# microsoft/ptgnn

Hardware: AMD Instinct MI355X
Metric: edges/sec per MP layer (higher is better)
Workload: dtype f32; 1 GPU; cfg3: Graph2Class-style batch, 48 graphs N=115772, T0=8->T=17, E=625130 (incl. reverse+self), Typilus GGNN arch: 8 GGNN layers H=128 (+concat residual), max; hidden=128, mode=forward (inference), fp32, plan_build_in_step=True, message_rows=shared per (edge type, source) pair, parallelism=single GPU, minibatches_rotated=4

## Files before the change

include/ptgnn_amd.h:

```cpp
#ifndef PTGNN_AMD_H_
#define PTGNN_AMD_H_

#include <stddef.h>
#include <stdint.h>

#ifdef __cplusplus
extern "C" {
#endif

#pragma GCC visibility push(default)

#define PTGNN_AMD_VERSION 102

enum {
  PTGNN_AMD_OK = 0,
  PTGNN_AMD_EINVAL = -1,
  PTGNN_AMD_EUNSUPPORTED = -2,
  PTGNN_AMD_EHIP = -3,
  PTGNN_AMD_EWORKSPACE = -4,
  PTGNN_AMD_ERANGE = -5
};

enum { PTGNN_AMD_SUM = 0, PTGNN_AMD_MEAN = 1, PTGNN_AMD_MAX = 2, PTGNN_AMD_MIN = 3 };

// ... 103 lines not shown
int64_t ptgnn_amd_hub_ticket_count(int64_t num_edges, int32_t msg_dim);
int ptgnn_amd_gather_reduce_f32(const float *ysrc, int64_t ld_ysrc,
                                const float *ydst , int64_t ld_ydst,
                                const int32_t *rowptr, const int32_t *col,
                                int32_t type_bits, int64_t num_nodes, int32_t msg_dim,
                                int reduce, int epilogue, const float *ln_gamma,
                                const float *ln_beta, float ln_eps, float *out, int64_t ld_out,
                                int32_t *argout , int64_t num_edges,
                                int32_t hub_threshold, const int32_t *hub_entries ,
                                const int32_t *hub_count , void *hub_ws ,
                                size_t hub_ws_bytes, int32_t *hub_tickets ,
                                void *stream);
int ptgnn_amd_gather_reduce_rows_f32(const float *ysrc, int64_t ld_ysrc,
                                     const float *ydst , int64_t ld_ydst,
                                     const int32_t *rowptr, const int32_t *col,
                                     int32_t type_bits, int64_t num_nodes, int32_t msg_dim,
                                     int reduce, int epilogue, const float *ln_gamma,
                                     const float *ln_beta, float ln_eps, float *out, int64_t ld_out,
                                     int32_t *argout , int64_t num_edges,
                                     int32_t hub_threshold, const int32_t *hub_entries ,
                                     const int32_t *hub_count , void *hub_ws ,
                                     size_t hub_ws_bytes, int32_t *hub_tickets ,
                                     int64_t row_begin, int64_t row_end, void *stream);

int ptgnn_amd_gather_update_supported(int32_t msg_dim, int32_t out_dim);
int ptgnn_amd_gather_update_f32(const float *msg, int64_t ld_msg, const int32_t *rowptr, const int32_t *col,
                                int32_t type_bits, int64_t num_nodes, int32_t msg_dim, int reduce, int epilogue,
                                const float *ln_gamma , const float *ln_beta , float ln_eps,
                                const float *w , const float *bias ,
                                int32_t out_dim, int act, float *out, int64_t ld_out, void *stream);

int ptgnn_amd_segment_mul_f32(const float *msg, int64_t ld_msg, const int32_t *rowptr, const int32_t *perm,
                              int64_t num_rows, int64_t num_edges, int32_t dim, float *out, int64_t ld_out,
                              void *stream);

int ptgnn_amd_gather_reduce_masked_f32(const float *grad, int64_t ld_grad, const int32_t *arg,
                                       const int32_t *rowptr, const int32_t *col,
                                       const int32_t *slot_of, int64_t num_rows, int32_t msg_dim,
                                       float *out, int64_t ld_out, int64_t num_edges,
                                       int32_t hub_threshold, const int32_t *hub_entries,
                                       const int32_t *hub_count, void *hub_ws ,
                                       size_t hub_ws_bytes, int32_t *hub_tickets ,
                                       void *stream);

int ptgnn_amd_linear_f32(const float *x, int64_t rows, int32_t k, int64_t ld_x, const float *w,
                         int32_t n_out, const float *bias, int act, float *y, int64_t ld_y,
// ... 250 lines not shown
```

ptgnn_amd/_lib.py:

```python
import ctypes
import os
import threading

import torch

_HERE = os.path.dirname(os.path.abspath(__file__))
LIB_PATH = os.environ.get("PTGNN_AMD_LIB") or os.path.join(_HERE, "csrc", "libptgnn_amd.so")

_c = ctypes
_i64, _i32, _vp, _f32 = _c.c_int64, _c.c_int32, _c.c_void_p, _c.c_float

SIGNATURES = {
    "ptgnn_amd_version": (_c.c_int, []),
    "ptgnn_amd_last_error": (_c.c_char_p, []),
    "ptgnn_amd_set_gemm_mode": (_c.c_int, [_c.c_int]),
    "ptgnn_amd_get_gemm_mode": (_c.c_int, []),
    "ptgnn_amd_launch_count": (_i64, [_c.c_int]),
    "ptgnn_amd_launch_name": (_c.c_char_p, [_c.c_int]),
    "ptgnn_amd_csr_workspace_bytes": (_c.c_size_t, [_i64, _i64]),
    "ptgnn_amd_csr_control_bytes": (_c.c_size_t, []),
    "ptgnn_amd_set_plan_path": (_c.c_int, [_c.c_int]),
    "ptgnn_amd_type_bits": (_c.c_int, [_i32]),
    "ptgnn_amd_csr_build": (_c.c_int, [_vp, _vp, _vp, _i32, _i64, _i64, _c.c_int, _vp, _vp, _vp, _vp,
                                       _i32, _vp, _vp, _vp, _vp, _vp, _c.c_size_t, _vp]),
    "ptgnn_amd_hub_workspace_bytes": (_c.c_size_t, [_i64, _i32, _c.c_int]),
    "ptgnn_amd_hub_ticket_count": (_i64, [_i64, _i32]),
    "ptgnn_amd_hub_list": (_c.c_int, [_vp, _i64, _i32, _vp, _vp, _vp]),
    "ptgnn_amd_validate_indices": (_c.c_int, [_vp, _i64, _i64, _vp, _vp]),
    "ptgnn_amd_shard_index_workspace_bytes": (_c.c_size_t, [_i64]),
    "ptgnn_amd_shard_index": (_c.c_int, [_vp, _vp, _vp, _i32, _i64, _i64, _vp, _i32, _i64, _vp, _vp, _vp, _i64, _vp,
                                         _vp, _vp, _c.c_size_t, _vp]),
    "ptgnn_amd_unique_sources_workspace_bytes": (_c.c_size_t, [_i64, _i32]),
    "ptgnn_amd_edge_table_bytes": (_c.c_size_t, []),
    "ptgnn_amd_unique_sources": (_c.c_int, [_vp, _i64, _i32, _i32, _i64, _vp, _vp, _i64, _vp, _vp, _vp, _c.c_size_t,
                                            _vp]),
    "ptgnn_amd_edge_linear_shared_supported": (_c.c_int, [_i32, _i32, _i32]),
    "ptgnn_amd_edge_linear_shared_f32": (_c.c_int, [_vp, _i64, _i64, _i32, _vp, _vp, _i32, _i32, _c.c_int, _vp, _i64,
                                                    _vp]),
    "ptgnn_amd_gather_reduce_f32": (_c.c_int, [_vp, _i64, _vp, _i64, _vp, _vp, _i32, _i64, _i32, _c.c_int,
                                               _c.c_int, _vp, _vp, _f32, _vp, _i64, _vp, _i64, _i32, _vp,
                                               _vp, _vp, _c.c_size_t, _vp, _vp]),
    "ptgnn_amd_gather_reduce_rows_f32": (_c.c_int, [_vp, _i64, _vp, _i64, _vp, _vp, _i32, _i64, _i32, _c.c_int,
                                                    _c.c_int, _vp, _vp, _f32, _vp, _i64, _vp, _i64, _i32, _vp,
                                                    _vp, _vp, _c.c_size_t, _vp, _i64, _i64, _vp]),
    "ptgnn_amd_gather_update_supported": (_c.c_int, [_i32, _i32]),
    "ptgnn_amd_gather_update_f32": (_c.c_int, [_vp, _i64, _vp, _vp, _i32, _i64, _i32, _c.c_int, _c.c_int, _vp, _vp, _f32,
                                               _vp, _vp, _i32, _c.c_int, _vp, _i64, _vp]),
    "ptgnn_amd_gather_reduce_masked_f32": (_c.c_int, [_vp, _i64, _vp, _vp, _vp, _vp, _i64, _i32, _vp, _i64,
                                                      _i64, _i32, _vp, _vp, _vp, _c.c_size_t, _vp, _vp]),
    "ptgnn_amd_segment_mul_f32": (_c.c_int, [_vp, _i64, _vp, _vp, _i64, _i64, _i32, _vp, _i64, _vp]),
    "ptgnn_amd_linear_f32": (_c.c_int, [_vp, _i64, _i32, _i64, _vp, _i32, _vp, _c.c_int, _vp, _i64,
                                        _vp]),
    "ptgnn_amd_linear_add_f32": (_c.c_int, [_vp, _i64, _i32, _i64, _vp, _i32, _vp, _c.c_int, _vp, _i64, _vp, _i64,
                                            _vp]),
    "ptgnn_amd_batch_offsets_i64": (_c.c_int, [_vp, _i64, _vp, _vp, _i32, _i64, _vp, _vp]),
    "ptgnn_amd_edge_linear_f32": (_c.c_int, [_vp, _i64, _i64, _i32, _vp, _vp, _vp, _vp, _i32, _i32, _c.c_int, _vp,
                                             _i64, _vp]),
    "ptgnn_amd_edge_linear_feat_f32": (_c.c_int, [_vp, _i64, _i64, _i32, _vp, _vp, _vp, _i64, _i32, _vp, _vp, _i32, _i32,
                                                  _c.c_int, _vp, _i64, _vp]),
    "ptgnn_amd_edge_linear_dropout_f32": (_c.c_int, [_vp, _i64, _i64, _i32, _vp, _vp, _vp, _i32, _i32, _vp, _i64,
                                                     _c.c_int, _c.c_float, _c.c_uint64, _vp]),
    "ptgnn_amd_dropout_bitmask_bytes": (_c.c_size_t, [_i64, _i32]),
    "ptgnn_amd_dropout_bitmask": (_c.c_int, [_i64, _i32, _c.c_float, _c.c_uint64, _vp, _vp]),
    "ptgnn_amd_edge_linear_masked_supported": (_c.c_int, [_i32, _i32, _c.c_int]),
    "ptgnn_amd_edge_linear_masked_f32": (_c.c_int, [_vp, _i64, _i64, _i32, _vp, _vp, _vp, _i32, _i32, _vp, _i64,
                                                    _c.c_int, _c.c_float, _vp, _vp]),
    "ptgnn_amd_edge_weight_grad_masked_supported": (_c.c_int, [_i32, _i32]),
# ... 128 lines not shown
```

ptgnn_amd/csrc/gather_reduce.hip:

```cpp
#include "gather_reduce_core.h"

namespace ptgnn_amd {
namespace {
constexpr int kSidePool = 64;
std::mutex g_side_mu;
SideStream g_side[kSidePool];
int g_side_used = 0;

bool side_streams_enabled() {
  static const bool enabled = [] {
    const char *e = getenv("PTGNN_AMD_HUB_STREAM");
    return !(e && e[0] == '0');
  }();
  return enabled;
}
}

SideStream *side_stream(hipStream_t caller, bool may_create) {
  if (!side_streams_enabled()) return nullptr;
  int dev = 0;
  if (hipGetDevice(&dev) != hipSuccess) return nullptr;
  std::lock_guard<std::mutex> lock(g_side_mu);
  for (int i = 0; i < g_side_used; ++i)
    if (g_side[i].dev == dev && g_side[i].owner == caller) return &g_side[i];
// ... 121 lines not shown
                                           int32_t type_bits, int64_t num_nodes, int32_t msg_dim,
                                           int reduce, int epilogue, const float *ln_gamma,
                                           const float *ln_beta, float ln_eps, float *out,
                                           int64_t ld_out, int32_t *argout, int64_t num_edges,
                                           int32_t hub_threshold, const int32_t *hub_entries,
                                           const int32_t *hub_count, void *hub_ws,
                                           size_t hub_ws_bytes, int32_t *hub_tickets, void *stream_) {
  return ptgnn_amd_gather_reduce_rows_f32(ysrc, ld_y, ydst, ld_yd, rowptr, col, type_bits, num_nodes, msg_dim, reduce,
                                          epilogue, ln_gamma, ln_beta, ln_eps, out, ld_out, argout, num_edges,
                                          hub_threshold, hub_entries, hub_count, hub_ws, hub_ws_bytes, hub_tickets, 0,
                                          num_nodes, stream_);
}

extern "C" int ptgnn_amd_gather_reduce_rows_f32(const float *ysrc, int64_t ld_y, const float *ydst,
                                                int64_t ld_yd, const int32_t *rowptr, const int32_t *col,
                                                int32_t type_bits, int64_t num_nodes, int32_t msg_dim,
                                                int reduce, int epilogue, const float *ln_gamma,
                                                const float *ln_beta, float ln_eps, float *out,
                                                int64_t ld_out, int32_t *argout, int64_t num_edges,
                                                int32_t hub_threshold, const int32_t *hub_entries,
                                                const int32_t *hub_count, void *hub_ws,
                                                size_t hub_ws_bytes, int32_t *hub_tickets, int64_t row_begin,
                                                int64_t row_end, void *stream_) {
  hipStream_t stream = (hipStream_t)stream_;
  PTGNN_REQUIRE(num_nodes >= 0 && msg_dim > 0 && num_edges >= 0, PTGNN_AMD_EINVAL, "gather_reduce: bad sizes");
  PTGNN_REQUIRE(row_begin >= 0 && row_begin <= row_end && row_end <= num_nodes, PTGNN_AMD_EINVAL,
                "gather_reduce: row range [%lld, %lld) outside [0, %lld]", (long long)row_begin, (long long)row_end,
                (long long)num_nodes);
  if (row_begin == row_end) return PTGNN_AMD_OK;
  PTGNN_REQUIRE(reduce >= PTGNN_AMD_SUM && reduce <= PTGNN_AMD_MIN, PTGNN_AMD_EINVAL,
                "gather_reduce: unknown reduce %d", reduce);
  PTGNN_REQUIRE(epilogue >= 0 && epilogue <= 3, PTGNN_AMD_EINVAL, "gather_reduce: bad epilogue");
  PTGNN_REQUIRE(type_bits >= 0 && type_bits < 16, PTGNN_AMD_EINVAL, "gather_reduce: bad type_bits");
  if (num_nodes == 0) return PTGNN_AMD_OK;
  PTGNN_REQUIRE(rowptr && out && ld_out >= msg_dim, PTGNN_AMD_EINVAL, "gather_reduce: null/ld");
  PTGNN_REQUIRE(col && (ysrc || num_edges == 0), PTGNN_AMD_EINVAL, "gather_reduce: null ysrc/col");
  PTGNN_REQUIRE(!(epilogue & PTGNN_AMD_EPI_LAYERNORM) || (ln_gamma && ln_beta), PTGNN_AMD_EINVAL,
                "gather_reduce: LayerNorm epilogue needs gamma/beta");
  PTGNN_REQUIRE(argout == nullptr || reduce >= PTGNN_AMD_MAX, PTGNN_AMD_EINVAL,
                "gather_reduce: argout only with max/min");

  Args a{};
  a.ysrc = ysrc; a.ydst = ydst; a.ld_y = ld_y; a.ld_yd = ydst ? ld_yd : ld_y;
  a.rowptr = rowptr; a.col = col; a.type_bits = type_bits; a.num_nodes = row_end; a.row_begin = row_begin; a.msg_dim = msg_dim;
  a.ln_gamma = ln_gamma; a.ln_beta = ln_beta; a.ln_eps = ln_eps; a.out = out; a.ld_out = ld_out;
  a.argout = argout; a.epi = epilogue;
  const int rc = setup_hub(a, num_edges, hub_threshold, hub_entries, hub_count, hub_ws, hub_ws_bytes,
                           hub_tickets, argout != nullptr);
  if (rc != PTGNN_AMD_OK) return rc;
  const bool vec4 = (msg_dim % 4 == 0) && (ld_y % 4 == 0) && (!ydst || ld_yd % 4 == 0) && (ld_out % 4 == 0) &&
                    aligned16(ysrc) && aligned16(out) && (!ydst || aligned16(ydst)) &&
                    (!argout || aligned16(argout));
  const bool row_epi = (epilogue & PTGNN_AMD_EPI_LAYERNORM) != 0;
  const int rc2 = dispatch_geometry(vec4, msg_dim, row_epi, [&](auto V, auto L, auto C, int col_blocks) {
    return launch1<decltype(V)::value, decltype(L)::value, decltype(C)::value>(a, reduce, col_blocks, stream);
  });
  if (rc2 == PTGNN_AMD_OK) count_launch(PTGNN_AMD_KERNEL_GATHER_REDUCE);
  return rc2;
}

extern "C" int ptgnn_amd_gather_update_supported(int32_t msg_dim, int32_t out_dim) {
  return msg_dim == kUpdM && out_dim >= 32 && out_dim <= 128 && out_dim % 32 == 0 ? 1 : 0;
}

extern "C" int ptgnn_amd_gather_update_f32(const float *msg, int64_t ld_msg, const int32_t *rowptr, const int32_t *col,
                                           int32_t type_bits, int64_t num_nodes, int32_t msg_dim, int reduce,
                                           int epilogue, const float *ln_gamma, const float *ln_beta, float ln_eps,
                                           const float *w, const float *bias, int32_t out_dim, int act, float *out,
                                           int64_t ld_out, void *stream_) {
// ... 45 lines not shown
  hipStream_t stream = (hipStream_t)stream_;
  PTGNN_REQUIRE(num_rows >= 0 && msg_dim > 0 && num_edges >= 0, PTGNN_AMD_EINVAL,
                "gather_reduce_masked: bad sizes");
  if (num_rows == 0) return PTGNN_AMD_OK;
  PTGNN_REQUIRE(grad && arg && rowptr && col && slot_of && out && ld_out >= msg_dim && ld_grad >= msg_dim,
                PTGNN_AMD_EINVAL, "gather_reduce_masked: null/ld");
  Args a{};
  a.ysrc = grad; a.ld_y = ld_grad; a.ld_yd = ld_grad; a.rowptr = rowptr; a.col = col;
  a.num_nodes = num_rows; a.msg_dim = msg_dim; a.out = out; a.ld_out = ld_out;
  a.mask_arg = arg; a.mask_slot = slot_of;
  const int rc = setup_hub(a, num_edges, hub_threshold, hub_entries, hub_count, hub_ws, hub_ws_bytes,
                           hub_tickets, false);
  if (rc != PTGNN_AMD_OK) return rc;
  const bool vec4 = (msg_dim % 4 == 0) && (ld_grad % 4 == 0) && (ld_out % 4 == 0) && aligned16(grad) &&
                    aligned16(out) && aligned16(arg);
  return dispatch_geometry(vec4, msg_dim, false, [&](auto V, auto L, auto C, int col_blocks) {
    return launch_all<decltype(V)::value, decltype(L)::value, decltype(C)::value, PTGNN_AMD_SUM, false, false,
                      true>(a, col_blocks, stream);
  });
}

namespace ptgnn_amd {
namespace {
__global__ __launch_bounds__(256) void k_gather_rows(const float *__restrict__ x, int64_t ld_x,
                                                     const int64_t *__restrict__ idx,
                                                     int64_t n_idx, int dim,
                                                     float *__restrict__ out, int64_t ld_out,
                                                     int vec4) {
  const int lane = threadIdx.x & 63;
  const int64_t w = (blockIdx.x * (int64_t)blockDim.x + threadIdx.x) >> 6;
  const int64_t nw = ((int64_t)gridDim.x * blockDim.x) >> 6;
  for (int64_t r = w; r < n_idx; r += nw) {
    const float *src = x + idx[r] * ld_x;
    float *dst = out + r * ld_out;
    if (vec4) {
      for (int c = lane * 4; c < dim; c += 256)
        *reinterpret_cast<float4 *>(dst + c) = *reinterpret_cast<const float4 *>(src + c);
    } else {
      for (int c = lane; c < dim; c += 64) dst[c] = src[c];
    }
  }
}
}
}

extern "C" int ptgnn_amd_gather_rows_f32(const float *x, int64_t ld_x, const int64_t *idx,
// ... 128 lines not shown
```

ptgnn_amd/csrc/gather_reduce_core.h:

```cpp
#pragma once
#include <float.h>
#include <stdlib.h>

#include <type_traits>

#include <mutex>

#include "dense_common.h"

namespace ptgnn_amd {

struct SideStream {
  int dev = -1;
  hipStream_t owner = nullptr;
  hipStream_t stream = nullptr;
  hipStream_t stream2 = nullptr;
  hipEvent_t fork = nullptr, join = nullptr, join2 = nullptr;
  std::mutex mu;
};

SideStream *side_stream(hipStream_t caller, bool may_create);

namespace {

constexpr int kHubChunk = 1024;
constexpr int kLongRow = 256;

struct Args {
  const float *ysrc;
  const float *ydst;
  int64_t ld_y;
  int64_t ld_yd;
  const int32_t *rowptr;
  const int32_t *col;
  int32_t type_bits;
  int64_t num_nodes;
  int64_t row_begin;
  int32_t msg_dim;
  const float *ln_gamma;
  const float *ln_beta;
  float ln_eps;
  float *out;
  int64_t ld_out;
  int32_t *argout;
  int64_t num_tiles;
  int32_t epi;
  const int32_t *mask_arg;
  const int32_t *mask_slot;
  int32_t hub_threshold;
  int32_t long_threshold;
  int32_t hub_blocks;
  float *hub_part;
  int32_t *hub_arg;
  int32_t *hub_tickets;
  const int32_t *hub_entries;
  const int32_t *hub_count;
  int64_t num_edges;
// ... 194 lines not shown
        pk[u] = a.col[idx < last ? idx : last];
      }
#pragma unroll
      for (int u = 0; u < U; ++u) {
        const int idx = i + u * stride;
        const bool valid = idx < end;
        if constexpr (HAS_DST) {
#pragma unroll
          for (int c = 0; c < CH; ++c)
#pragma unroll
            for (int v = 0; v < VEC; ++v) m[u][c][v] += DST_ONCE ? d1[c][v] : d[DST_ONCE ? 0 : u][c][v];
        }
        if (REDUCE != PTGNN_AMD_MAX && REDUCE != PTGNN_AMD_MIN) {
#pragma unroll
          for (int c = 0; c < CH; ++c)
#pragma unroll
            for (int v = 0; v < VEC; ++v) m[u][c][v] = valid ? m[u][c][v] : 0.f;
        }
        fold(m[u], valid ? idx : last);
      }
    }
  }

  __device__ __forceinline__ void store(float *orow, int32_t *arow) const {
#pragma unroll
    for (int c = 0; c < CH; ++c) {
      const int colx = cbase + (g + c * LPR) * VEC;
      if (colx >= M) continue;
      if constexpr (VEC == 4) {
        *reinterpret_cast<float4 *>(orow + colx) = make_float4(acc[c][0], acc[c][1], acc[c][2], acc[c][3]);
        if (HAS_ARG) *reinterpret_cast<int4 *>(arow + colx) = make_int4(arg[c][0], arg[c][1], arg[c][2], arg[c][3]);
      } else {
        orow[colx] = acc[c][0];
        if (HAS_ARG) arow[colx] = arg[c][0];
      }
    }
  }

  __device__ __forceinline__ void finish_and_store(int64_t row, int deg) {
    finish(deg);
    if constexpr (COMB) combine_store(row);
    else store(a.out + row * a.ld_out, HAS_ARG ? a.argout + row * (int64_t)M : nullptr);
  }

  __device__ __forceinline__ void combine_store(int64_t row) {
    __shared__ __attribute__((aligned(16))) float stage[256 * VEC * CH];
// ... 180 lines not shown
      float m[FB][CH][VEC];
      int ma[FB][CH][VEC];
#pragma unroll
      for (int u = 0; u < FB; ++u) {
        const int64_t c = c0 + u <= c_last ? c0 + u : c_last;
        const int w2 = (c > c_first || rbeg == (int)(c_first * kHubChunk)) ? 0 : 1;
        fin.load_partial(a.hub_part + (2 * c + w2) * (int64_t)a.msg_dim,
                         HAS_ARG ? a.hub_arg + (2 * c + w2) * (int64_t)a.msg_dim : nullptr, m[u], ma[u]);
      }
#pragma unroll
      for (int u = 0; u < FB; ++u)
        if (c0 + u <= c_last) fin.fold_partial(m[u], ma[u]);
    }
    fin.finish_and_store(row, rend - rbeg);
  }
}

template <int VEC, int LPR, int CH, int REDUCE, bool HAS_DST, bool HAS_ARG, bool MASKED, bool COMB = false>
__global__ __launch_bounds__(256) void k_hub_chunks(Args a) {
  hub_chunks_body<VEC, LPR, CH, REDUCE, HAS_DST, HAS_ARG, MASKED, false, COMB>(a, (int)blockIdx.x, (int)gridDim.x);
}

template <int VEC, int LPR, int CH, int REDUCE, bool HAS_DST, bool HAS_ARG, bool MASKED, bool DST1 = false,
          bool HUBF = hub_fuses<CH, HAS_DST, HAS_ARG, MASKED>(), bool COMB = false>
__global__ __launch_bounds__(256) void k_gather_reduce(Args a) {
  constexpr int ROWS_PER_BLOCK = 256 / LPR;
  if constexpr (HUBF) {
    if ((int)blockIdx.x < a.hub_blocks) {
      hub_chunks_body<VEC, LPR, CH, REDUCE, HAS_DST, HAS_ARG, MASKED, true, COMB>(a, (int)blockIdx.x, a.hub_blocks);
      return;
    }
  }
  const int64_t tile = xcd_swizzle(blockIdx.x - a.hub_blocks, gridDim.x - a.hub_blocks);
  if (tile >= a.num_tiles) return;
  const int64_t row = a.row_begin + tile * ROWS_PER_BLOCK + threadIdx.x / LPR;
  if (row >= a.num_nodes) return;
  const int beg = a.rowptr[row], end = a.rowptr[row + 1];
  if (a.hub_threshold > 0 && end - beg > a.hub_threshold) return;
  if (a.long_threshold > 0 && end - beg > a.long_threshold) return;
  RowOp<VEC, LPR, CH, REDUCE, HAS_DST, HAS_ARG, MASKED, COMB> op(a, threadIdx.x % LPR,
                                                               blockIdx.y * (LPR * VEC * CH));
  constexpr int UP = (VEC == 4 && !MASKED && (!HAS_DST || DST1)) ? (CH == 1 ? 8 : 4) : 0;
  if constexpr (UP == 0) op.reduce(row, beg, end, 1);
  else op.template reduce_pf<UP, HAS_DST && DST1>(row, beg, end, 1);
  op.finish_and_store(row, end - beg);
}

template <int VEC, int LPR, int CH, int REDUCE, bool HAS_DST, bool HAS_ARG, bool COMB = false>
__global__ __launch_bounds__(256) void k_long_rows(Args a) {
  const int lane = threadIdx.x & 63;
  const int64_t wave = ((int64_t)blockIdx.x * 256 + threadIdx.x) >> 6;
  const int64_t nwaves = ((int64_t)gridDim.x * 256) >> 6;
  for (int64_t base = a.row_begin + wave * 64; base < a.num_nodes; base += nwaves * 64) {
    const int64_t r = base + lane;
    int beg = 0, deg = 0;
    if (r < a.num_nodes) {
      beg = a.rowptr[r];
      deg = a.rowptr[r + 1] - beg;
    }
    unsigned long long todo = __ballot(deg > a.long_threshold && deg <= a.hub_threshold);
    while (todo) {
      const int b = __ffsll((long long)todo) - 1;
      todo &= todo - 1;
      const int rbeg = __shfl(beg, b, 64), rdeg = __shfl(deg, b, 64);
      if (lane < LPR) {
        RowOp<VEC, LPR, CH, REDUCE, HAS_DST, HAS_ARG, false, COMB> op(a, lane, blockIdx.y * (LPR * VEC * CH));
        op.template reduce_pf<16, HAS_DST>(base + b, rbeg, rbeg + rdeg, 1);
        op.finish_and_store(base + b, rdeg);
      }
    }
  }
}

template <int VEC, int LPR, int CH, int REDUCE, bool HAS_DST, bool HAS_ARG, bool MASKED, bool COMB = false>
int launch_all(const Args &a0, int col_blocks, hipStream_t stream) {
  static_assert(!COMB || (!HAS_DST && !MASKED), "the EGC combine finishes plain rows");
  constexpr int ROWS_PER_BLOCK = 256 / LPR;
  Args a = a0;
  a.num_tiles = (a.num_nodes - a.row_begin + ROWS_PER_BLOCK - 1) / ROWS_PER_BLOCK;
  a.hub_blocks = 0;
  SideStream *side = nullptr;
  static const int64_t side_min_edges = [] {
    const char *e = getenv("PTGNN_AMD_SIDE_MIN_EDGES");
    return e ? (int64_t)atoll(e) : ((int64_t)1 << 21);
  }();
  if (a.hub_threshold > 0 && a.num_edges >= side_min_edges) {
    hipStreamCaptureStatus cs = hipStreamCaptureStatusNone;
    (void)hipStreamIsCapturing(stream, &cs);
    side = side_stream(stream, cs == hipStreamCaptureStatusNone);
  }
  bool long_launch = false;
  std::unique_lock<std::mutex> side_lock;
  if (side) side_lock = std::unique_lock<std::mutex>(side->mu);
  if (side) {
// ... 10 lines not shown
        long_launch = true;
        PTGNN_HIP(hipStreamWaitEvent(side->stream2, side->fork, 0));
        const int64_t lb = (a.num_nodes - a.row_begin + 255) / 256;
        dim3 lgrid((unsigned)(lb < 2048 ? lb : 2048), (unsigned)col_blocks);
        k_long_rows<VEC, LPR, CH, REDUCE, HAS_DST, HAS_ARG, COMB><<<lgrid, 256, 0, side->stream2>>>(a);
        PTGNN_LAUNCH_CHECK();
        PTGNN_HIP(hipEventRecord(side->join2, side->stream2));
      }
    }
  }
  constexpr bool kFuseHub = hub_fuses<CH, HAS_DST, HAS_ARG, MASKED>();
  constexpr bool kHubF = kFuseHub;
  constexpr bool kFuseSmall = hub_fuses_small<CH, HAS_DST, HAS_ARG, MASKED>();
  const bool fuse_small = kFuseSmall && a.num_edges < kFuseDstMaxEdges;
  if ((kFuseHub || fuse_small) && !side && a.hub_threshold > 0 && a.num_edges < side_min_edges) {
    const int64_t chunks = (a.num_edges + kHubChunk - 1) / kHubChunk;
    a.hub_blocks = (int)(((chunks < PTGNN_HUB_FUSED_BLOCKS ? chunks : PTGNN_HUB_FUSED_BLOCKS) + 7) / 8 * 8);
  }
  dim3 grid((unsigned)(xcd_padded_blocks(a.num_tiles) + a.hub_blocks), (unsigned)col_blocks);
  constexpr bool kDst1Variant = VEC == 4 && HAS_DST && !MASKED;
  if constexpr (kFuseSmall) {
    if (a.hub_blocks > 0) {
      if (kDst1Variant && a.type_bits == 0)
        k_gather_reduce<VEC, LPR, CH, REDUCE, HAS_DST, HAS_ARG, MASKED, kDst1Variant, true><<<grid, 256, 0, stream>>>(a);
      else
        k_gather_reduce<VEC, LPR, CH, REDUCE, HAS_DST, HAS_ARG, MASKED, false, true><<<grid, 256, 0, stream>>>(a);
      PTGNN_LAUNCH_CHECK();
      return PTGNN_AMD_OK;
    }
  }
  if (kDst1Variant && a.type_bits == 0)
    k_gather_reduce<VEC, LPR, CH, REDUCE, HAS_DST, HAS_ARG, MASKED, kDst1Variant, kHubF, COMB><<<grid, 256, 0, stream>>>(a);
  else
    k_gather_reduce<VEC, LPR, CH, REDUCE, HAS_DST, HAS_ARG, MASKED, false, kHubF, COMB><<<grid, 256, 0, stream>>>(a);
  PTGNN_LAUNCH_CHECK();
  if (side) {
    PTGNN_HIP(hipStreamWaitEvent(stream, side->join, 0));
    if (long_launch) PTGNN_HIP(hipStreamWaitEvent(stream, side->join2, 0));
    return PTGNN_AMD_OK;
  }
  if (a.hub_blocks == 0 && a.hub_threshold > 0) {
    int64_t chunks = (a.num_edges + kHubChunk - 1) / kHubChunk;
    dim3 hgrid((unsigned)(chunks < 1024 ? chunks : 1024), (unsigned)col_blocks);
    k_hub_chunks<VEC, LPR, CH, REDUCE, HAS_DST, HAS_ARG, MASKED, COMB><<<hgrid, 256, 0, stream>>>(a);
    PTGNN_LAUNCH_CHECK();
  }
  return PTGNN_AMD_OK;
}

template <int VEC, int LPR, int CH, int REDUCE, bool HAS_DST>
int launch2(const Args &a, int col_blocks, hipStream_t stream) {
  if constexpr (REDUCE == PTGNN_AMD_MAX || REDUCE == PTGNN_AMD_MIN) {
    if (a.argout) return launch_all<VEC, LPR, CH, REDUCE, HAS_DST, true, false>(a, col_blocks, stream);
  }
  return launch_all<VEC, LPR, CH, REDUCE, HAS_DST, false, false>(a, col_blocks, stream);
}

// ... 69 lines not shown
```

ptgnn_amd/ops.py:

```python
import ctypes
import os
import weakref
from typing import List, Optional, Sequence, Tuple

import torch

from ptgnn_amd import _lib
from ptgnn_amd._readback import LOCK, Backoff, Readback, take_arrived

REDUCE_IDS = {"sum": 0, "add": 0, "mean": 1, "max": 2, "min": 3}
EPI_NONE, EPI_GELU, EPI_LAYERNORM, EPI_GELU_LAYERNORM = 0, 1, 2, 3
ACT_IDS = {None: 0, "none": 0, "tanh": 1, "relu": 2}


GEMM_MODES = {"tile": 0, "stream": 1}


def set_gemm_mode(mode) -> int:
    lib = _lib.load()
    prev = lib.ptgnn_amd_get_gemm_mode()
    if isinstance(mode, str) and mode not in GEMM_MODES:
        raise _lib.PtgnnAmdError(f"unknown GEMM mode {mode!r} (have {sorted(GEMM_MODES)}; the split mode was removed)")
    _lib.check(lib.ptgnn_amd_set_gemm_mode(int(GEMM_MODES.get(mode, mode))), "ptgnn_amd_set_gemm_mode")
    return prev
# ... 122 lines not shown
        self.bad_ids = self.bad_readback = self.side_stream = None
        self.uniq_backoff, self.uniq_pending = Backoff(), []
        self.hub_backoff, self.hub_pending = Backoff(), []
        self.plan_control = {}


_STATES = {}


def _device_state(device) -> _DeviceState:
    key = torch.device(device).index or 0
    st = _STATES.get(key)
    if st is None:
        with LOCK:
            st = _STATES.setdefault(key, _DeviceState(key))
    return st


class GraphPlan:

    __slots__ = ("rowptr", "col", "perm", "type_bits", "num_nodes", "num_edges", "num_types",
                 "num_src_rows", "_backward", "_adj", "_adj_refs", "_inv_perm", "_ready", "_waited",
                 "_hub_tickets", "hub_entries", "hub_count", "_slot_rows", "_ident", "_transposed", "_uniq", "_hub_posted",
                 "_has_hubs", "__weakref__")

    def __init__(self, rowptr, col, perm, type_bits, num_nodes, num_edges, num_types):
        self.rowptr, self.col, self.perm = rowptr, col, perm
        self.type_bits, self.num_nodes = type_bits, num_nodes
        self.num_edges, self.num_types = num_edges, num_types
        self.num_src_rows = num_nodes
        self._backward = None
        self._adj = None
        self._adj_refs = None
        self._inv_perm = None
        self._ready = None
        self._waited = set()
        self._hub_tickets = {}
        self.hub_entries = self.hub_count = None
        self._slot_rows = self._ident = self._transposed = None
        self._uniq = None
        self._hub_posted = False
        self._has_hubs = None

    def may_have_hubs(self) -> bool:
        return self.hub_entries is not None

    def hub_tickets(self, msg_dim: int) -> torch.Tensor:
        n = _lib.load().ptgnn_amd_hub_ticket_count(self.num_edges, msg_dim)
        dev = self.rowptr.device
        key = (n, torch.cuda.current_stream(dev).cuda_stream)
        t = self._hub_tickets.get(key)
        if t is None:
            t = torch.zeros(max(n, 1), dtype=torch.int32, device=dev)
            self._hub_tickets[key] = t
        return t

    def wait(self) -> None:
        if self._ready is not None:
            cur = torch.cuda.current_stream(self.rowptr.device)
            if cur.cuda_stream not in self._waited:
                cur.wait_event(self._ready)
                self._waited.add(cur.cuda_stream)

    def unique_messages(self) -> Optional["UniqueMessages"]:
        if self._uniq is None:
            self._uniq = _launch_unique_sources(self) or False
        return self._uniq or None

    def backward_plan(self) -> "GraphPlan":
        if self._backward is None:
            if self._adj is None:
                raise _lib.PtgnnAmdError("this plan was built without keeping its adjacency lists")
            self.wait()
            self._backward = build_plan(self._adj, self.num_src_rows * self.num_types, mode=2)
        return self._backward

    def forward_slot_of_backward_slot(self) -> torch.Tensor:
        bp = self.backward_plan()
        if bp._inv_perm is None:
            inv = self.inverse_perm()
            bp._inv_perm = inv[bp.perm[: self.num_edges].to(torch.int64)].to(torch.int32).contiguous()
        return bp._inv_perm

    def slot_rows(self) -> torch.Tensor:
        if self._slot_rows is None:
# ... 17 lines not shown
            self._ident = out
        return self._ident

    def transposed_plan(self) -> "GraphPlan":
        if self._transposed is None:
            if self._adj is None:
                raise _lib.PtgnnAmdError("this plan was built without keeping its adjacency lists")
            self.wait()
            self._transposed = build_plan(self._adj, self.num_src_rows, mode=1)
        return self._transposed

    def inverse_perm(self) -> torch.Tensor:
        if self._inv_perm is None:
            self.wait()
            inv = torch.empty(max(self.num_edges, 1), dtype=torch.int64, device=self.perm.device)
            inv[self.perm[: self.num_edges].to(torch.int64)] = torch.arange(
                self.num_edges, device=self.perm.device)
            self._inv_perm = inv
        return self._inv_perm


class UniqueMessages:
    __slots__ = ("slot_row", "unique_src", "edge_table", "capacity", "counts", "num_edges", "num_types", "_readback",
                 "_counts")

    def __init__(self, slot_row, unique_src, edge_table, capacity, counts, num_edges, num_types):
        self.slot_row, self.unique_src, self.edge_table = slot_row, unique_src, edge_table
        self.capacity, self.counts, self.num_edges, self.num_types = capacity, counts, num_edges, num_types
        self._readback = self._counts = None

    def host_counts(self, wait: bool = False) -> Optional[List[int]]:
        if self._counts is None:
            if self._readback is not None:
                self._counts = self._readback.values(wait)
            elif wait:
                self._counts = [int(c) for c in self.counts.tolist()]
        return self._counts

    def rows(self, wait: bool = False) -> Optional[int]:
        c = self.host_counts(wait)
        return None if c is None else c[self.num_types]

    def adjacency(self):
        adj, off = [], 0
        for c in self.host_counts(wait=True)[:-1]:
            adj.append((self.unique_src[off: off + c], self.unique_src[off: off + c]))
            off += c
        return adj


UNIQUE_MIN_SAVING = float(os.environ.get("PTGNN_AMD_UNIQUE_MIN_SAVING", "0.05"))
UNIQUE_MIN_EDGES = int(os.environ.get("PTGNN_AMD_UNIQUE_MIN_EDGES", "65536"))
# ... 18 lines not shown
    if not capturing:
        _poll_unique_stats(st)
        if st.uniq_backoff.consume():
            return None
    plan.wait()
    cap = max(1, min(E, ns * T))
    slot_row = torch.empty(max(E, 1), dtype=torch.int32, device=dev)
    unique_src = torch.empty(cap, dtype=torch.int64, device=dev)
    counts = torch.empty(T + 1, dtype=torch.int64, device=dev)
    table = torch.empty(int(lib.ptgnn_amd_edge_table_bytes()), dtype=torch.uint8, device=dev)
    ws_bytes = int(lib.ptgnn_amd_unique_sources_workspace_bytes(ns, T))
    ws = _workspace(ws_bytes, dev)
    with _timed("unique_sources", bytes=E * 12.0 + ns * T / 4.0):
        rc = lib.ptgnn_amd_unique_sources(plan.col.data_ptr(), E, plan.type_bits, T, ns, slot_row.data_ptr(),
                                          unique_src.data_ptr(), cap, counts.data_ptr(), table.data_ptr(),
                                          ws.data_ptr(), ws_bytes, _stream(slot_row))
    _lib.check(rc, "ptgnn_amd_unique_sources")
    u = UniqueMessages(slot_row, unique_src, table, cap, counts, E, T)
    if not capturing:
        u._readback = Readback(counts, tag=(E, T))
        with LOCK:
            st.uniq_pending.append(u._readback)
    return u


def edge_linear_shared_supported(state_dim: int, msg_dim: int, num_types: int) -> bool:
    return bool(_lib.load().ptgnn_amd_edge_linear_shared_supported(state_dim, msg_dim, num_types))


def edge_linear_shared(x: torch.Tensor, uniq: UniqueMessages, weights: Sequence[torch.Tensor],
                       act: Optional[str] = None) -> torch.Tensor:
    lib = _lib.load()
    _require_cuda_f32("x", x)
    x = _rowmajor(x)
    T, H, M = uniq.num_types, x.shape[1], weights[0].shape[0]
    if len(weights) != T:
        raise _lib.PtgnnAmdError(f"edge_linear_shared: {len(weights)} weights for {T} edge types")
    ws = [w.detach().contiguous() for w in weights]
    for w in ws:
        if tuple(w.shape) != (M, H) or not w.is_cuda or w.dtype != torch.float32:
            raise _lib.PtgnnAmdError(f"edge_linear_shared: weight shape {tuple(w.shape)} does not match [{M}, {H}]")
    msg = torch.empty(uniq.capacity, M, dtype=torch.float32, device=x.device)
    wp = (ctypes.c_void_p * T)(*[w.data_ptr() for w in ws])

    def rows():
        r = uniq.rows(wait=True)
# ... 294 lines not shown
    N = plan.num_nodes
    caller_out = out
    if out is None:
        out = torch.empty(N, msg_dim, dtype=torch.float32, device=ysrc.device)
    elif tuple(out.shape) != (N, msg_dim) or out.dtype != torch.float32 or not out.is_contiguous():
        raise _lib.PtgnnAmdError(f"gather_reduce: `out` must be a contiguous float32 [{N}, {msg_dim}] tensor")
    arg = None
    if return_arg:
        arg = torch.empty(N, msg_dim, dtype=torch.int32, device=ysrc.device)
    if epilogue & EPI_LAYERNORM:
        ln_weight, ln_bias = ln_weight.contiguous(), ln_bias.contiguous()
    plan.wait()
    tb, colt = _slot_map(plan, type_bits, col)
    nbytes = (plan.num_edges * (4.0 * msg_dim + 4) + N * (4.0 * msg_dim + 4)
              + (N * 4.0 * msg_dim if ydst is not None else 0.0)
              + (N * 4.0 * msg_dim if arg is not None else 0.0))
    lo, hi = (0, N) if rows is None else (int(rows[0]), int(rows[1]))
    if rows is not None:
        if caller_out is None or return_arg:
            raise _lib.PtgnnAmdError("gather_reduce: a row range needs a caller-owned `out` (the other rows are not "
                                     "written) and returns no arg")
        nbytes *= (hi - lo) / max(N, 1)
    hub_ws, hub = _hub_args(plan, msg_dim, arg is not None, ysrc.device)
    with _timed("gather_reduce", bytes=nbytes):
        rc = lib.ptgnn_amd_gather_reduce_rows_f32(
            _ptr_or(ysrc, plan.rowptr), ld_y, ydst.data_ptr() if ydst is not None else None, ld_yd,
            plan.rowptr.data_ptr(), colt.data_ptr(), tb, N, msg_dim,
            REDUCE_IDS[reduce], epilogue,
            ln_weight.data_ptr() if ln_weight is not None else None,
            ln_bias.data_ptr() if ln_bias is not None else None, float(ln_eps),
            out.data_ptr(), msg_dim, arg.data_ptr() if arg is not None else None,
            *hub, lo, hi, _stream(out))
    _lib.check(rc, "ptgnn_amd_gather_reduce_rows_f32")
    return (out, arg) if return_arg else out


GATHER_UPDATE = os.environ.get("PTGNN_AMD_GATHER_UPDATE", "1") not in ("", "0")
GATHER_UPDATE_MAX_EDGES = 1 << 21


GATHER_UPDATE_BACKOFF = 64


def _poll_hub_counts(st: _DeviceState) -> None:
    for readback in take_arrived(st.hub_pending, keep=16):
        hubs = readback.values()[0] > 0
        plan = readback.tag()
        if plan is not None:
            plan._has_hubs = hubs
        if hubs:
            st.hub_backoff.trip(GATHER_UPDATE_BACKOFF)


def gather_update_supported(msg_dim: int, out_dim: int, plan: "GraphPlan") -> bool:
    if not (GATHER_UPDATE and plan.num_edges < GATHER_UPDATE_MAX_EDGES
            and bool(_lib.load().ptgnn_amd_gather_update_supported(int(msg_dim), int(out_dim)))):
# ... 1350 lines not shown
```

Baseline: 1.291 billion edges/s.

## Precompute per-row 8-entry column headers for aligned vector loads in gather-reduce

Adds a kernel that builds, once per plan and entry array, a 32-byte-aligned header per destination row holding its first 8 column entries (padded with the last one). The plain float4 gather-reduce walk then loads those 8 source indices with two vector loads instead of scattered col reads, which shortens the dependent latency chain before the message row gathers begin. Headers are cached on the plan (and on the unique-message slot map), so they are built once per plan and reused across layers. The cost is an extra N*32-byte buffer, one additional kernel launch per plan, and more template instantiations.

```diff
diff --git a/include/ptgnn_amd.h b/include/ptgnn_amd.h
--- a/include/ptgnn_amd.h
+++ b/include/ptgnn_amd.h
@@ -149,6 +149,19 @@
                                      const int32_t *hub_count , void *hub_ws ,
                                      size_t hub_ws_bytes, int32_t *hub_tickets ,
                                      int64_t row_begin, int64_t row_end, void *stream);
+int ptgnn_amd_row_headers(const int32_t *rowptr, const int32_t *entries, int64_t num_rows, int32_t *hdr, void *stream);
+int ptgnn_amd_gather_reduce_hdr_f32(const float *ysrc, int64_t ld_ysrc,
+                                    const float *ydst , int64_t ld_ydst,
+                                    const int32_t *rowptr, const int32_t *col,
+                                    int32_t type_bits, int64_t num_nodes, int32_t msg_dim,
+                                    int reduce, int epilogue, const float *ln_gamma,
+                                    const float *ln_beta, float ln_eps, float *out, int64_t ld_out,
+                                    int32_t *argout , int64_t num_edges,
+                                    int32_t hub_threshold, const int32_t *hub_entries ,
+                                    const int32_t *hub_count , void *hub_ws ,
+                                    size_t hub_ws_bytes, int32_t *hub_tickets ,
+                                    int64_t row_begin, int64_t row_end,
+                                    const int32_t *row_hdr , void *stream);
 
 int ptgnn_amd_gather_update_supported(int32_t msg_dim, int32_t out_dim);
 int ptgnn_amd_gather_update_f32(const float *msg, int64_t ld_msg, const int32_t *rowptr, const int32_t *col,
diff --git a/ptgnn_amd/_lib.py b/ptgnn_amd/_lib.py
--- a/ptgnn_amd/_lib.py
+++ b/ptgnn_amd/_lib.py
@@ -43,6 +43,10 @@
     "ptgnn_amd_gather_reduce_rows_f32": (_c.c_int, [_vp, _i64, _vp, _i64, _vp, _vp, _i32, _i64, _i32, _c.c_int,
                                                     _c.c_int, _vp, _vp, _f32, _vp, _i64, _vp, _i64, _i32, _vp,
                                                     _vp, _vp, _c.c_size_t, _vp, _i64, _i64, _vp]),
+    "ptgnn_amd_row_headers": (_c.c_int, [_vp, _vp, _i64, _vp, _vp]),
+    "ptgnn_amd_gather_reduce_hdr_f32": (_c.c_int, [_vp, _i64, _vp, _i64, _vp, _vp, _i32, _i64, _i32, _c.c_int,
+                                                   _c.c_int, _vp, _vp, _f32, _vp, _i64, _vp, _i64, _i32, _vp,
+                                                   _vp, _vp, _c.c_size_t, _vp, _i64, _i64, _vp, _vp]),
     "ptgnn_amd_gather_update_supported": (_c.c_int, [_i32, _i32]),
     "ptgnn_amd_gather_update_f32": (_c.c_int, [_vp, _i64, _vp, _vp, _i32, _i64, _i32, _c.c_int, _c.c_int, _vp, _vp, _f32,
                                                _vp, _vp, _i32, _c.c_int, _vp, _i64, _vp]),
diff --git a/ptgnn_amd/csrc/gather_reduce.hip b/ptgnn_amd/csrc/gather_reduce.hip
--- a/ptgnn_amd/csrc/gather_reduce.hip
+++ b/ptgnn_amd/csrc/gather_reduce.hip
@@ -167,8 +167,25 @@
                                                 const int32_t *hub_count, void *hub_ws,
                                                 size_t hub_ws_bytes, int32_t *hub_tickets, int64_t row_begin,
                                                 int64_t row_end, void *stream_) {
+  return ptgnn_amd_gather_reduce_hdr_f32(ysrc, ld_y, ydst, ld_yd, rowptr, col, type_bits, num_nodes, msg_dim, reduce,
+                                         epilogue, ln_gamma, ln_beta, ln_eps, out, ld_out, argout, num_edges,
+                                         hub_threshold, hub_entries, hub_count, hub_ws, hub_ws_bytes, hub_tickets,
+                                         row_begin, row_end, nullptr, stream_);
+}
+
+extern "C" int ptgnn_amd_gather_reduce_hdr_f32(const float *ysrc, int64_t ld_y, const float *ydst,
+                                               int64_t ld_yd, const int32_t *rowptr, const int32_t *col,
+                                               int32_t type_bits, int64_t num_nodes, int32_t msg_dim,
+                                               int reduce, int epilogue, const float *ln_gamma,
+                                               const float *ln_beta, float ln_eps, float *out,
+                                               int64_t ld_out, int32_t *argout, int64_t num_edges,
+                                               int32_t hub_threshold, const int32_t *hub_entries,
+                                               const int32_t *hub_count, void *hub_ws,
+                                               size_t hub_ws_bytes, int32_t *hub_tickets, int64_t row_begin,
+                                               int64_t row_end, const int32_t *row_hdr, void *stream_) {
   hipStream_t stream = (hipStream_t)stream_;
   PTGNN_REQUIRE(num_nodes >= 0 && msg_dim > 0 && num_edges >= 0, PTGNN_AMD_EINVAL, "gather_reduce: bad sizes");
+  PTGNN_REQUIRE(((uintptr_t)row_hdr & 31) == 0, PTGNN_AMD_EINVAL, "gather_reduce: row_hdr must be 32-byte aligned");
   PTGNN_REQUIRE(row_begin >= 0 && row_begin <= row_end && row_end <= num_nodes, PTGNN_AMD_EINVAL,
                 "gather_reduce: row range [%lld, %lld) outside [0, %lld]", (long long)row_begin, (long long)row_end,
                 (long long)num_nodes);
@@ -190,6 +207,7 @@
   a.rowptr = rowptr; a.col = col; a.type_bits = type_bits; a.num_nodes = row_end; a.row_begin = row_begin; a.msg_dim = msg_dim;
   a.ln_gamma = ln_gamma; a.ln_beta = ln_beta; a.ln_eps = ln_eps; a.out = out; a.ld_out = ld_out;
   a.argout = argout; a.epi = epilogue;
+  a.hdr = row_hdr;
   const int rc = setup_hub(a, num_edges, hub_threshold, hub_entries, hub_count, hub_ws, hub_ws_bytes,
                            hub_tickets, argout != nullptr);
   if (rc != PTGNN_AMD_OK) return rc;
@@ -281,6 +299,35 @@
 
 namespace ptgnn_amd {
 namespace {
+__global__ __launch_bounds__(256) void k_row_headers(const int32_t *__restrict__ rowptr,
+                                                     const int32_t *__restrict__ entries, int64_t num_rows,
+                                                     int32_t *__restrict__ hdr) {
+  const int64_t i = (int64_t)blockIdx.x * 256 + threadIdx.x;
+  const int64_t r = i >> 3;
+  if (r >= num_rows) return;
+  const int k = (int)(i & 7);
+  const int beg = rowptr[r], end = rowptr[r + 1];
+  int32_t v = 0;
+  if (end > beg) v = entries[beg + k < end ? beg + k : end - 1];
+  hdr[i] = v;
+}
+}
+}
+
+extern "C" int ptgnn_amd_row_headers(const int32_t *rowptr, const int32_t *entries, int64_t num_rows, int32_t *hdr,
+                                     void *stream_) {
+  PTGNN_REQUIRE(num_rows >= 0 && num_rows < ((int64_t)1 << 31), PTGNN_AMD_EINVAL, "row_headers: bad sizes");
+  if (num_rows == 0) return PTGNN_AMD_OK;
+  PTGNN_REQUIRE(rowptr && entries && hdr, PTGNN_AMD_EINVAL, "row_headers: null pointer");
+  PTGNN_REQUIRE(((uintptr_t)hdr & 31) == 0, PTGNN_AMD_EINVAL, "row_headers: hdr must be 32-byte aligned");
+  const int64_t blocks = (num_rows * 8 + 255) / 256;
+  k_row_headers<<<(unsigned)blocks, 256, 0, (hipStream_t)stream_>>>(rowptr, entries, num_rows, hdr);
+  PTGNN_LAUNCH_CHECK();
+  return PTGNN_AMD_OK;
+}
+
+namespace ptgnn_amd {
+namespace {
 __global__ __launch_bounds__(256) void k_gather_rows(const float *__restrict__ x, int64_t ld_x,
                                                      const int64_t *__restrict__ idx,
                                                      int64_t n_idx, int dim,
diff --git a/ptgnn_amd/csrc/gather_reduce_core.h b/ptgnn_amd/csrc/gather_reduce_core.h
--- a/ptgnn_amd/csrc/gather_reduce_core.h
+++ b/ptgnn_amd/csrc/gather_reduce_core.h
@@ -33,6 +33,7 @@
   int64_t ld_yd;
   const int32_t *rowptr;
   const int32_t *col;
+  const int32_t *hdr;
   int32_t type_bits;
   int64_t num_nodes;
   int64_t row_begin;
@@ -273,6 +274,51 @@
     }
   }
 
+  template <int U>
+  __device__ __forceinline__ void reduce_hdr(int beg, int end, const int32_t (&first)[U]) {
+    static_assert(VEC == 4 && !MASKED && !HAS_ARG && !HAS_DST, "the header walk serves plain float4 rows");
+    if (beg >= end) return;
+    fold_group<U>(first, beg, end);
+    for (int i = beg + U; i < end; i += U) {
+      int32_t pk[U];
+#pragma unroll
+      for (int u = 0; u < U; ++u) pk[u] = a.col[i + u < end ? i + u : end - 1];
+      fold_group<U>(pk, i, end);
+    }
+  }
+
+  template <int U>
+  __device__ __forceinline__ void fold_group(const int32_t (&pk)[U], int i, int end) {
+    constexpr bool kMinMax = REDUCE == PTGNN_AMD_MAX || REDUCE == PTGNN_AMD_MIN;
+    float m[U][CH][VEC];
+#pragma unroll
+    for (int u = 0; u < U; ++u) {
+      const int64_t s = pk[u] >> a.type_bits;
+      const int t = pk[u] & tmask;
+      const float *base = a.ysrc + s * a.ld_y + (int64_t)t * M;
+#pragma unroll
+      for (int c = 0; c < CH; ++c) {
+        const int colx = cbase + (g + c * LPR) * VEC;
+        if (colx < M && i + u < end) {
+          const float4 v = *reinterpret_cast<const float4 *>(base + colx);
+          m[u][c][0] = v.x; m[u][c][1] = v.y; m[u][c][2] = v.z; m[u][c][3] = v.w;
+        } else {
+#pragma unroll
+          for (int v = 0; v < VEC; ++v) m[u][c][v] = 0.f;
+        }
+      }
+    }
+#pragma unroll
+    for (int u = 0; u < U; ++u) {
+      const bool valid = i + u < end;
+#pragma unroll
+      for (int c = 0; c < CH; ++c)
+#pragma unroll
+        for (int v = 0; v < VEC; ++v) m[u][c][v] = valid ? m[u][c][v] : (kMinMax ? kInit : 0.f);
+      fold(m[u], i + u);
+    }
+  }
+
   __device__ __forceinline__ void store(float *orow, int32_t *arow) const {
 #pragma unroll
     for (int c = 0; c < CH; ++c) {
@@ -499,7 +545,7 @@
 }
 
 template <int VEC, int LPR, int CH, int REDUCE, bool HAS_DST, bool HAS_ARG, bool MASKED, bool DST1 = false,
-          bool HUBF = hub_fuses<CH, HAS_DST, HAS_ARG, MASKED>(), bool COMB = false>
+          bool HUBF = hub_fuses<CH, HAS_DST, HAS_ARG, MASKED>(), bool COMB = false, bool HDR = false>
 __global__ __launch_bounds__(256) void k_gather_reduce(Args a) {
   constexpr int ROWS_PER_BLOCK = 256 / LPR;
   if constexpr (HUBF) {
@@ -512,13 +558,29 @@
   if (tile >= a.num_tiles) return;
   const int64_t row = a.row_begin + tile * ROWS_PER_BLOCK + threadIdx.x / LPR;
   if (row >= a.num_nodes) return;
-  const int beg = a.rowptr[row], end = a.rowptr[row + 1];
+  constexpr int UP = (VEC == 4 && !MASKED && (!HAS_DST || DST1)) ? (CH == 1 ? 8 : 4) : 0;
+  static_assert(!HDR || UP == 8, "row headers serve the walks in groups of 8");
+  int32_t pk[HDR ? 8 : 1];
+  int beg, end;
+  if constexpr (HDR) {
+    typedef int32_t i32x4 __attribute__((ext_vector_type(4)));
+    const i32x4 *rec = reinterpret_cast<const i32x4 *>(a.hdr + row * 8);
+    i32x4 h0 = rec[0], h1 = rec[1];
+    beg = a.rowptr[row];
+    end = a.rowptr[row + 1];
+    asm volatile("" : "+v"(h0), "+v"(h1), "+v"(beg), "+v"(end));
+    pk[0] = h0.x; pk[1] = h0.y; pk[2] = h0.z; pk[3] = h0.w;
+    pk[4] = h1.x; pk[5] = h1.y; pk[6] = h1.z; pk[7] = h1.w;
+  } else {
+    beg = a.rowptr[row];
+    end = a.rowptr[row + 1];
+  }
   if (a.hub_threshold > 0 && end - beg > a.hub_threshold) return;
   if (a.long_threshold > 0 && end - beg > a.long_threshold) return;
   RowOp<VEC, LPR, CH, REDUCE, HAS_DST, HAS_ARG, MASKED, COMB> op(a, threadIdx.x % LPR,
                                                                blockIdx.y * (LPR * VEC * CH));
-  constexpr int UP = (VEC == 4 && !MASKED && (!HAS_DST || DST1)) ? (CH == 1 ? 8 : 4) : 0;
   if constexpr (UP == 0) op.reduce(row, beg, end, 1);
+  else if constexpr (HDR) op.template reduce_hdr<8>(beg, end, pk);
   else op.template reduce_pf<UP, HAS_DST && DST1>(row, beg, end, 1);
   op.finish_and_store(row, end - beg);
 }
@@ -547,6 +609,22 @@
       }
     }
   }
+}
+
+template <int VEC, int CH, bool HAS_DST, bool HAS_ARG, bool MASKED, bool COMB>
+constexpr bool hdr_walk() {
+  return VEC == 4 && CH == 1 && !MASKED && !COMB && !HAS_ARG && !HAS_DST;
+}
+
+template <int VEC, int LPR, int CH, int REDUCE, bool HAS_DST, bool HAS_ARG, bool MASKED, bool DST1, bool HUBF, bool COMB>
+void launch_main(const Args &a, dim3 grid, hipStream_t stream) {
+  if constexpr (hdr_walk<VEC, CH, HAS_DST, HAS_ARG, MASKED, COMB>()) {
+    if (a.hdr != nullptr) {
+      k_gather_reduce<VEC, LPR, CH, REDUCE, HAS_DST, HAS_ARG, MASKED, DST1, HUBF, COMB, true><<<grid, 256, 0, stream>>>(a);
+      return;
+    }
+  }
+  k_gather_reduce<VEC, LPR, CH, REDUCE, HAS_DST, HAS_ARG, MASKED, DST1, HUBF, COMB, false><<<grid, 256, 0, stream>>>(a);
 }
 
 template <int VEC, int LPR, int CH, int REDUCE, bool HAS_DST, bool HAS_ARG, bool MASKED, bool COMB = false>
@@ -603,17 +681,17 @@
   if constexpr (kFuseSmall) {
     if (a.hub_blocks > 0) {
       if (kDst1Variant && a.type_bits == 0)
-        k_gather_reduce<VEC, LPR, CH, REDUCE, HAS_DST, HAS_ARG, MASKED, kDst1Variant, true><<<grid, 256, 0, stream>>>(a);
+        launch_main<VEC, LPR, CH, REDUCE, HAS_DST, HAS_ARG, MASKED, kDst1Variant, true, false>(a, grid, stream);
       else
-        k_gather_reduce<VEC, LPR, CH, REDUCE, HAS_DST, HAS_ARG, MASKED, false, true><<<grid, 256, 0, stream>>>(a);
+        launch_main<VEC, LPR, CH, REDUCE, HAS_DST, HAS_ARG, MASKED, false, true, false>(a, grid, stream);
       PTGNN_LAUNCH_CHECK();
       return PTGNN_AMD_OK;
     }
   }
   if (kDst1Variant && a.type_bits == 0)
-    k_gather_reduce<VEC, LPR, CH, REDUCE, HAS_DST, HAS_ARG, MASKED, kDst1Variant, kHubF, COMB><<<grid, 256, 0, stream>>>(a);
+    launch_main<VEC, LPR, CH, REDUCE, HAS_DST, HAS_ARG, MASKED, kDst1Variant, kHubF, COMB>(a, grid, stream);
   else
-    k_gather_reduce<VEC, LPR, CH, REDUCE, HAS_DST, HAS_ARG, MASKED, false, kHubF, COMB><<<grid, 256, 0, stream>>>(a);
+    launch_main<VEC, LPR, CH, REDUCE, HAS_DST, HAS_ARG, MASKED, false, kHubF, COMB>(a, grid, stream);
   PTGNN_LAUNCH_CHECK();
   if (side) {
     PTGNN_HIP(hipStreamWaitEvent(stream, side->join, 0));
diff --git a/ptgnn_amd/ops.py b/ptgnn_amd/ops.py
--- a/ptgnn_amd/ops.py
+++ b/ptgnn_amd/ops.py
@@ -168,7 +168,7 @@
     __slots__ = ("rowptr", "col", "perm", "type_bits", "num_nodes", "num_edges", "num_types",
                  "num_src_rows", "_backward", "_adj", "_adj_refs", "_inv_perm", "_ready", "_waited",
                  "_hub_tickets", "hub_entries", "hub_count", "_slot_rows", "_ident", "_transposed", "_uniq", "_hub_posted",
-                 "_has_hubs", "__weakref__")
+                 "_has_hubs", "_hdrs", "__weakref__")
 
     def __init__(self, rowptr, col, perm, type_bits, num_nodes, num_edges, num_types):
         self.rowptr, self.col, self.perm = rowptr, col, perm
@@ -187,6 +187,7 @@
         self._uniq = None
         self._hub_posted = False
         self._has_hubs = None
+        self._hdrs = {}
 
     def may_have_hubs(self) -> bool:
         return self.hub_entries is not None
@@ -207,6 +208,25 @@
             if cur.cuda_stream not in self._waited:
                 cur.wait_event(self._ready)
                 self._waited.add(cur.cuda_stream)
+
+    def row_header(self, entries: Optional[torch.Tensor] = None) -> Optional[torch.Tensor]:
+        if self._adj is None:
+            return None
+        uniq = self._uniq or None
+        if entries is None or entries is self.col:
+            key, entries = "col", self.col
+        elif entries is self.perm:
+            key = "perm"
+        elif uniq is not None and entries is uniq.slot_row:
+            if uniq.hdr is None:
+                uniq.hdr = _launch_row_headers(self, entries)
+            return uniq.hdr
+        else:
+            return None
+        hdr = self._hdrs.get(key)
+        if hdr is None:
+            hdr = self._hdrs[key] = _launch_row_headers(self, entries)
+        return hdr
 
     def unique_messages(self) -> Optional["UniqueMessages"]:
         if self._uniq is None:
@@ -270,12 +290,12 @@
 
 class UniqueMessages:
     __slots__ = ("slot_row", "unique_src", "edge_table", "capacity", "counts", "num_edges", "num_types", "_readback",
-                 "_counts")
+                 "_counts", "hdr")
 
     def __init__(self, slot_row, unique_src, edge_table, capacity, counts, num_edges, num_types):
         self.slot_row, self.unique_src, self.edge_table = slot_row, unique_src, edge_table
         self.capacity, self.counts, self.num_edges, self.num_types = capacity, counts, num_edges, num_types
-        self._readback = self._counts = None
+        self._readback = self._counts = self.hdr = None
 
     def host_counts(self, wait: bool = False) -> Optional[List[int]]:
         if self._counts is None:
@@ -340,6 +360,20 @@
         with LOCK:
             st.uniq_pending.append(u._readback)
     return u
+
+
+ROW_HEADERS = os.environ.get("PTGNN_AMD_ROW_HEADERS", "1") not in ("", "0")
+
+
+def _launch_row_headers(plan: "GraphPlan", entries: torch.Tensor) -> torch.Tensor:
+    N = plan.num_nodes
+    plan.wait()
+    hdr = torch.empty(max(N, 1), 8, dtype=torch.int32, device=plan.rowptr.device)
+    with _timed("row_headers", bytes=N * (32.0 + 4) + 4.0 * min(plan.num_edges, 8 * N)):
+        rc = _lib.load().ptgnn_amd_row_headers(plan.rowptr.data_ptr(), entries.data_ptr(), N, hdr.data_ptr(),
+                                               _stream(hdr))
+    _lib.check(rc, "ptgnn_amd_row_headers")
+    return hdr
 
 
 def edge_linear_shared_supported(state_dim: int, msg_dim: int, num_types: int) -> bool:
@@ -680,16 +714,20 @@
                                      "written) and returns no arg")
         nbytes *= (hi - lo) / max(N, 1)
     hub_ws, hub = _hub_args(plan, msg_dim, arg is not None, ysrc.device)
+    hdr = None
+    if (ROW_HEADERS and ydst is None and arg is None and msg_dim % 4 == 0 and msg_dim <= 256 and ld_y % 4 == 0
+            and ysrc.data_ptr() % 16 == 0 and out.data_ptr() % 16 == 0):
+        hdr = plan.row_header(colt)
     with _timed("gather_reduce", bytes=nbytes):
-        rc = lib.ptgnn_amd_gather_reduce_rows_f32(
+        rc = lib.ptgnn_amd_gather_reduce_hdr_f32(
             _ptr_or(ysrc, plan.rowptr), ld_y, ydst.data_ptr() if ydst is not None else None, ld_yd,
             plan.rowptr.data_ptr(), colt.data_ptr(), tb, N, msg_dim,
             REDUCE_IDS[reduce], epilogue,
             ln_weight.data_ptr() if ln_weight is not None else None,
             ln_bias.data_ptr() if ln_bias is not None else None, float(ln_eps),
             out.data_ptr(), msg_dim, arg.data_ptr() if arg is not None else None,
-            *hub, lo, hi, _stream(out))
-    _lib.check(rc, "ptgnn_amd_gather_reduce_rows_f32")
+            *hub, lo, hi, hdr.data_ptr() if hdr is not None else None, _stream(out))
+    _lib.check(rc, "ptgnn_amd_gather_reduce_hdr_f32")
     return (out, arg) if return_arg else out
 
 
```

New measurement: 1.322 billion edges/s (median of 6 runs). 2.3% higher.
